# NCKempke/PIPS-IPMpp

Measured on AMD Instinct MI355X. Metric: KKT factor+solve per IPM iter/sec, N-block arrowhead LP, higher is better.
Workload: dtype f64; 1 GPU; 64 blocks x 10000 vars (5000 eq rows, rho=0.001), Schur dim 2000, 64 blocks/GPU [BASELINE configs[1]]; deterministic=False, family=random, root=dense LDL^T, sparse_head=multifrontal (k_front), solves_per_unit=4, collective=none, nnzL_per_gpu=649118456

## Files before the change

include/pips_hip.h:

```cpp
#ifndef PIPS_HIP_H
#define PIPS_HIP_H
#include <stddef.h>
#include <stdint.h>

#ifdef __cplusplus
extern "C" {
#endif

const char* pips_hip_last_error(void);
long long pips_hip_host_wait_count(void);
int pips_hip_host_wait_sites(char* buf, int cap);
long long pips_hip_device_allocs_live(void);
long long pips_hip_device_bytes_live(void);
int pips_hip_device_count(void);

int pips_hip_ldl_create(void** handle, int n, const int* krow, const int* jcol, int device, int flags);
int pips_hip_ldl_set_inertia_hint(void* handle, int n_primal);
int pips_hip_ldl_set_pivot_rule(void* handle, double thr_rel, double repl_rel);
int pips_hip_ldl_set_refinement(void* handle, int max_steps, double tol);
int pips_hip_ldl_set_refinement_backward_error(void* handle, int max_steps, double tol);
int pips_hip_ldl_set_deterministic(void* handle, int on);
int pips_hip_ldl_analyze(void* handle);
int pips_hip_ldl_factor(void* handle, const double* vals_host);
int pips_hip_ldl_solve(void* handle, int nrhs, double* rhs_inout_host, int ld);
// ... 197 lines not shown
int pips_gen_root(uint64_t seed, int n0, int myl, int* F0_rowptr, int* F0_colidx, double* F0_val, double* c0,
                  double* xstar0);
int pips_gen_diagonal(uint64_t seed, int block, int n, double lo, double hi, double* d);
int pips_kkt_leaf_assemble(int nx, int my, int mz, const int* Q_rowptr, const int* Q_colidx, const double* Q_val,
                           const int* B_rowptr, const int* B_colidx, const double* B_val, const int* D_rowptr,
                           const int* D_colidx, const double* D_val, int* K_rowptr, int* K_colidx, double* K_val,
                           int* diag_pos);
int pips_border_assemble(int nx, int my, int mz, int n0, int n_empty, int myl, int mzl, const int* R_rowptr,
                         const int* R_colidx, const double* R_val, const int* A_rowptr, const int* A_colidx,
                         const double* A_val, const int* C_rowptr, const int* C_colidx, const double* C_val,
                         const int* F_rowptr, const int* F_colidx, const double* F_val, const int* G_rowptr,
                         const int* G_colidx, const double* G_val, int* Bt_rowptr, int* Bt_colidx, double* Bt_val);
int pips_map_children_to_ranks(int n_children, int n_ranks, int* map);
int pips_symbolic_probe(int n, int n_primal, const int* krow, const int* jcol, int S, const int* Bt_rowptr,
                        const int* Bt_colidx, int force_n_head, int64_t* what, int n_what, int* perm, int* colcount);

int pips_symbolic_probe_hubs(int n, int n_primal, const int* krow, const int* jcol, int n_hubs, const int* hubs, int min_size,
                             int64_t* what, int n_what, int* perm, int* colcount);

int pips_layout_probe(int nblk, const int* n, const int* n_primal, const int* const* krow, const int* const* kcol,
                      int S, const int* const* bt_rowptr, const int* const* bt_colidx,
                      int deterministic, long long free_device_bytes, int64_t* what, int n_what);

int pips_schur_pack_probe(int nblk, int S, const int* const* bt_rowptr, int* nb, int* nb_max, int* const* local_of_row);

int pips_gdx_read_block(void** block, const char* path, int num_blocks, int act_block, int offset);
int pips_gdx_block_counts(void* block, long long* counts14);
int pips_gdx_block_vector(void* block, int which, double* out, int capacity, int* length);
int pips_gdx_block_matrix(void* block, int which, int* present, int* rows, int* cols, int* rowptr, int* colidx, double* val);
void pips_gdx_block_destroy(void* block);

#ifdef __cplusplus
}
#endif
#endif
```

pips-ipmpp_amd/csrc/engine.hip:

```cpp
#include <hip/hip_runtime.h>

#include <algorithm>
#include <cstdlib>
#include <cstring>
#include <map>
#include <memory>
#include <mutex>
#include <thread>
#include <vector>

#include "common.h"
#include "devmem.h"
#include "layout.h"
#include "kernels.hip.h"
#include "rootkernel.hip.h"
#include "tailkernel.hip.h"
#include "pips_hip.h"

namespace pips {

static thread_local std::string g_last_error;
void set_last_error(const std::string& msg) { g_last_error = msg; }
std::atomic<long long> g_host_waits{0};
struct WaitSite { std::atomic<const char*> file{nullptr}; std::atomic<int> line{0}; std::atomic<long long> n{0}; };
// ... 35 lines not shown
static int env_flag(const char* name) {
   const char* v = getenv(name);
   return v ? (atoi(v) != 0 ? 1 : 0) : -1;
}

static inline int grid_for(long long n, int block, int cap = 4096) {
   long long g = (n + block - 1) / block;
   if (g < 1) g = 1;
   if (g > cap) g = cap;
   return (int)g;
}

struct TaskList { long long off = 0; int cnt = 0; };

struct TailPlan {
   int ntc_max = 0;
   std::vector<TaskList> upd, upd_diag, diag, trsm, fwd, bwd, trail, trail_next;
   TaskList schur;
   DevBuf<TileTask> d_tasks;
   std::vector<TileTask> h_tasks;

   int build(const std::vector<BlkDesc>& blks, int panel = 0, bool lookahead = false, bool split_diag = false,
             const std::vector<const std::vector<int>*>* first = nullptr, bool diag_ahead = false, int pair2 = 1) {
      std::vector<TileTask> all;
      ntc_max = 0;
      for (auto& b : blks) ntc_max = std::max(ntc_max, b.ntc);
      upd.assign(ntc_max, {});
      upd_diag.assign(ntc_max, {});
      diag.assign(ntc_max, {});
      trsm.assign(ntc_max, {});
      fwd.assign(ntc_max, {});
      bwd.assign(ntc_max, {});
      trail.assign(ntc_max, {});
      trail_next.assign(ntc_max, {});
      const int nblk = (int)blks.size();
      auto begin = [&](TaskList& l) { l.off = (long long)all.size(); };
      auto end = [&](TaskList& l) { l.cnt = (int)((long long)all.size() - l.off); };
      for (int j = 0; j < ntc_max; ++j) {
         const int p0 = panel > 0 ? j / panel * panel : 0;
         auto fst = [&](int b, int t) { return first ? (*(*first)[b])[t] : 0; };
         begin(upd_diag[j]);
         if (j > p0 && split_diag)
            for (int b = 0; b < nblk; ++b)
               if (blks[b].ntc > j) {
                  const int k0 = std::max(p0, fst(b, j));
                  if (k0 < j) all.push_back({b, j, j, (diag_ahead ? std::max(k0, j - 1) : k0) | (j << 16)});
// ... 54 lines not shown
         end(bwd[j]);
         if (panel > 0 && (j + 1) % panel == 0) {
            begin(trail_next[j]);
            if (lookahead)
               for (int b = 0; b < nblk; ++b)
                  if (j + 1 < blks[b].ntc)
                     for (int ti = j + 1; ti < blks[b].ntr; ++ti) all.push_back({b, ti, j + 1, p0 | ((j + 1) << 16)});
            end(trail_next[j]);
            begin(trail[j]);
            for (int b = 0; b < nblk; ++b)
               for (int tj = j + (lookahead ? 2 : 1); tj < blks[b].ntc; ++tj)
                  for (int ti = tj; ti < blks[b].ntr; ++ti) all.push_back({b, ti, tj, p0 | ((j + 1) << 16)});
            end(trail[j]);
         }
      }
      begin(schur);
      for (int b = 0; b < nblk; ++b)
         if (blks[b].ntc > 0 && blks[b].nb > 0) {
            const int nt = blks[b].nb_pad / TILE;
            for (int ti = 0; ti < nt; ++ti)
               for (int tj = 0; tj <= ti; ++tj) all.push_back({b, ti, tj, 0});
         }
      end(schur);
      h_tasks = all;
      return d_tasks.upload(all);
   }
};

struct SweepRt {
   DevBuf<TileTask> d_tasks;
   int n_tasks = 0;
   DevBuf<int> d_ints;
   long long n_flags = 0;
   DevBuf<long long> d_flag_off, d_tfirst_off;
   DevBuf<int> d_tfirst;
   int epoch = 0;
   bool enabled = false;
   long long poll_limit = SWEEP_POLL_LIMIT;
   int take_error(const char* who) {
      if (!d_ints) return PIPS_OK;
      int w = 0;
      HIP_TRY(hipMemcpy(&w, d_ints + 2 * SWEEP_NRHS_MAX, sizeof(int), hipMemcpyDeviceToHost));
      if (!w) return PIPS_OK;
      HIP_TRY(hipMemset(d_ints + 2 * SWEEP_NRHS_MAX, 0, sizeof(int)));
      PIPS_FAIL(PIPS_ERR_HIP, "%s: a single-launch solve sweep gave up waiting for a piece of the solution after %lld polls (its output is NaN); "
                              "another process holding the device for seconds can cause that - PIPS_HIP_SWEEP_LAUNCHES=1 selects the launch-per-column sweeps",
                who, poll_limit);
   }
// ... 185 lines not shown
   bool is_root = false;
   const int* d_sctab = nullptr;
   const std::vector<TaskList>* sc_groups = nullptr;
   const TileTask* d_sc_tasks = nullptr;
   const std::vector<hipEvent_t>* ev_sc = nullptr;
   int* d_ctr_pool = nullptr;
   int* ctr_cursor = nullptr;
   const std::vector<TaskList>* det_rounds = nullptr;
   const TileTask* d_det_tasks = nullptr;
   double* d_gbuf = nullptr;
   long long gstride = 0;
   const int* d_blk_group = nullptr;
   int n_groups = 0, first_slot = 0;
   long long sc_len = 0;
   bool det_defer_reduce = false;
   bool det_reduce_later = false;
   bool bunch_kaufman = false;
   int *d_pert_cnt = nullptr, *d_pert_list = nullptr;
   const double* bk_orig = nullptr;
   int bk_orig_ld = 0, bk_orig_rowmajor = 0;
   const int* d_bk_perm = nullptr;
   int bk_isolate = 0;
   const TailSingle* single = nullptr;
};
constexpr int GEMM_CTR_SLOTS = 4096;
constexpr int GEMM_BAL_MIN_TASKS = 1024;

static void reduce_det_groups(const TailCtx& c, double* SC, int ldSC) {
   const int S_ = ldSC;
   if (c.det_defer_reduce) {
   } else if (c.d_sctab)
      hipLaunchKernelGGL(k_reduce_groups, dim3((unsigned)std::max(1LL, std::min(1024LL, (c.sc_len + 255) / 256)), 1), dim3(256), 0, c.stream, SC, 0, (int)c.sc_len,
                         c.d_gbuf, c.gstride, c.n_groups, c.first_slot);
   else
      hipLaunchKernelGGL(k_reduce_groups, dim3(std::max(1, std::min(64, (S_ + 255) / 256)), S_), dim3(256), 0, c.stream, SC, ldSC, S_, c.d_gbuf,
                         c.gstride, c.n_groups, c.first_slot);
}

static inline int tile_grid(int n) { return (n + 7) / 8 * 8; }
template <int MODE>
static void launch_tile_gemm(const TailCtx& c, const TileTask* tasks, const TaskList& l, hipStream_t st, double* SC = nullptr, int ldSC = 0) {
   const bool rounds = MODE == 2 && c.det_rounds;
   hipLaunchKernelGGL(k_tile_gemm<MODE>, dim3(tile_grid(l.cnt)), dim3(512), 0, st, tasks + l.off, l.cnt, c.d_blks, c.d_arena, c.d_dtail, c.d_winv, c.d_bmap, SC, ldSC,
                      MODE == 2 ? c.d_sctab : nullptr, c.d_uarena, rounds ? c.d_gbuf : nullptr, rounds ? c.gstride : 0, rounds ? c.d_blk_group : nullptr);
}
static bool tile_gemm_bal_ready(const TailCtx& c) { return c.d_ctr_pool && *c.ctr_cursor < GEMM_CTR_SLOTS; }
template <int MODE>
static void launch_tile_gemm_bal(const TailCtx& c, const TileTask* tasks, const TaskList& l, hipStream_t st, double* SC = nullptr, int ldSC = 0) {
   const int wgs = tile_grid(l.cnt) / 8 * 9;
   hipLaunchKernelGGL(k_tile_gemm_bal<MODE>, dim3(tile_grid(wgs)), dim3(512), 0, st, tasks + l.off, l.cnt, c.d_blks, c.d_arena, c.d_dtail, c.d_winv, c.d_bmap, SC, ldSC,
                      MODE == 2 ? c.d_sctab : nullptr, c.d_uarena, c.d_ctr_pool + 8 * (*c.ctr_cursor)++);
}
static void launch_tile_diag(const TailCtx& c, const TileTask* tasks, const TaskList& l, hipStream_t st) {
   if (c.bunch_kaufman)
      hipLaunchKernelGGL(k_tile_diag_bk, dim3(l.cnt), dim3(256), 0, st, tasks + l.off, c.d_blks, c.d_arena, c.d_dtail, c.d_winv, c.d_inertia, c.d_pert_cnt, c.d_pert_list,
                         c.bk_orig, c.bk_orig_ld, c.bk_orig_rowmajor, c.d_bk_perm, c.bk_isolate);
   else
      hipLaunchKernelGGL(k_tile_diag, dim3(l.cnt), dim3(256), 0, st, tasks + l.off, c.d_blks, c.d_arena, c.d_dtail, c.d_winv, c.d_psign, c.d_psign_off, c.d_inertia, c.d_pref);
}
static void launch_tile_update(const TailCtx& c, const TaskList& l, hipStream_t st) {
   if (!c.is_root && l.cnt >= GEMM_BAL_MIN_TASKS && tile_gemm_bal_ready(c))
      launch_tile_gemm_bal<0>(c, c.plan->d_tasks, l, st);
   else if (c.is_root)
      launch_tile_gemm<3>(c, c.plan->d_tasks, l, st);
   else
      launch_tile_gemm<0>(c, c.plan->d_tasks, l, st);
}

static int dump_tail_trace(const TailCtx& c, DevBuf<long long>& d_trace, size_t n_trace, const char* trace_file) {
   const TailSingle& ts = *c.single;
   std::vector<long long> h(n_trace);
   std::vector<TileTask> ht((size_t)ts.n_tasks);
   HIP_TRY(hipStreamSynchronize(c.stream));
   HIP_TRY(hipMemcpy(h.data(), d_trace, h.size() * sizeof(long long), hipMemcpyDeviceToHost));
   HIP_TRY(hipMemcpy(ht.data(), ts.d_tasks, ht.size() * sizeof(TileTask), hipMemcpyDeviceToHost));
   d_trace.reset();
   if (FILE* f = fopen(trace_file, "w")) {
      for (int t = 0; t < ts.n_tasks; ++t) {
         int x = 0;
         while (x < 7 && t >= ts.args.xoff[x + 1]) ++x;
         fprintf(f, "%d %d %d %d %d %d %d %lld %lld %lld\n", t, x, ht[t].blk >> 24, ht[t].blk & 0xffffff, ht[t].ti, ht[t].tj, ht[t].pad, h[3 * (size_t)t], h[3 * (size_t)t + 1],
                 h[3 * (size_t)t + 2]);
      }
      fclose(f);
   }
   return PIPS_OK;
}

static int tail_single_launch(const TailCtx& c) {
// ... 51 lines not shown
         else launch_tile_gemm<1>(c, p.d_tasks, p.trsm[j], c.stream);
      }
      if (p.trsm[j].cnt > 0 && c.bunch_kaufman && c.is_root && c.d_pert_cnt)
         hipLaunchKernelGGL(k_bk_growth, dim3(TILE), dim3(256), 0, c.stream, c.d_blks, c.d_arena, j, 1e8, c.d_pert_cnt, c.d_pert_list);
      if (p.trail_next[j].cnt > 0 || p.trail[j].cnt > 0) {
         PIPS_TRY(main_writes(j + 1));
         const bool split = c.side && p.trail[j].cnt > 0;
         if (split) {
            HIP_TRY(hipEventRecord(c.ev_panel, c.stream));
            HIP_TRY(hipStreamWaitEvent(c.side, c.ev_panel, 0));
            launch_tile_update(c, p.trail[j], c.side);
            HIP_TRY(hipEventRecord(c.ev_rest, c.side));
            side_busy = true;
            side_from = j + 2;
         }
         PhaseTimer::Scope phase(c.timer, c.stream, 2);
         if (p.trail_next[j].cnt > 0) launch_tile_update(c, p.trail_next[j], c.stream);
         if (!split && p.trail[j].cnt > 0) launch_tile_update(c, p.trail[j], c.stream);
      }
   }
   return main_writes(1 << 30);
}

static int tail_schur(const TailCtx& c, double* SC, int ldSC) {
   const TailPlan& p = *c.plan;
   const bool rounds = c.det_rounds != nullptr, panels = !rounds && c.sc_groups && !c.d_sctab;
   if (!SC || (!rounds && !panels && p.schur.cnt == 0)) return PIPS_OK;
   PhaseTimer::Scope phase(c.timer, c.stream, 5);
   if (rounds) {
      for (const TaskList& l : *c.det_rounds)
         if (l.cnt > 0) launch_tile_gemm<2>(c, c.d_det_tasks, l, c.stream, SC, ldSC);
      if (!c.det_reduce_later) reduce_det_groups(c, SC, ldSC);
   } else if (panels) {
      for (size_t g = 0; g < c.sc_groups->size(); ++g) {
         const TaskList& l = (*c.sc_groups)[g];
         if (l.cnt > 0) launch_tile_gemm<2>(c, c.d_sc_tasks, l, c.stream, SC, ldSC);
         HIP_TRY(hipEventRecord((*c.ev_sc)[g], c.stream));
      }
   } else if (tile_gemm_bal_ready(c) && !c.d_sctab)
      launch_tile_gemm_bal<2>(c, p.d_tasks, p.schur, c.stream, SC, ldSC);
   else
      launch_tile_gemm<2>(c, p.d_tasks, p.schur, c.stream, SC, ldSC);
   return PIPS_OK;
}

static int tail_factor(const TailCtx& c, double* SC, int ldSC) {
   const bool trsm_tri = !c.bunch_kaufman && !c.is_root && env_int("PIPS_HIP_TRSM_DENSE", 0) == 0;
   if (!c.single) PIPS_TRY(tail_columns(c, trsm_tri));
   else if (c.single->n_tasks > 0) PIPS_TRY(tail_single_launch(c));
   PIPS_TRY(tail_schur(c, SC, ldSC));
   HIP_TRY(hipGetLastError());
   return PIPS_OK;
}

static int tail_fwd(const TailCtx& c, double* xw, int nrhs = 1, long long xw_stride = 0) {
   const TailPlan& p = *c.plan;
   if (c.sweep && c.sweep->enabled && nrhs <= SWEEP_NRHS_MAX) {
      hipLaunchKernelGGL(k_tail_rows_fwd, dim3(c.sweep->n_tasks, nrhs), dim3(256), 0, c.stream, c.sweep->args(xw_stride, c.stream), c.d_blks, c.d_arena, c.d_dtail,
                         c.d_winv, xw);
      HIP_TRY(hipGetLastError());
      return PIPS_OK;
   }
   for (int j = 0; j < p.ntc_max; ++j)
      if (p.fwd[j].cnt > 0)
         hipLaunchKernelGGL(k_tail_fwd, dim3(p.fwd[j].cnt, nrhs), dim3(256), 0, c.stream, p.d_tasks + p.fwd[j].off, c.d_blks,
                            c.d_arena, c.d_dtail, c.d_winv, xw, j, xw_stride);
   HIP_TRY(hipGetLastError());
   return PIPS_OK;
}

static int tail_bwd(const TailCtx& c, double* xw, int nrhs = 1, long long xw_stride = 0, int border = 0) {
// ... 32 lines not shown
   SchurPack pack;
   int packed_rhs = 0;
   DevBuf<int> d_pk_la;
   DevBuf<long long> d_pk_tabrow;
   std::vector<int> h_pk_la, h_pk_tab;
   std::vector<long long> h_pk_tabrow;
   DevBuf<int> d_kb_rec;
   DevBuf<long long> d_kb_off;
   DevBuf<int> d_kb_list;
   DevBuf<int> d_kb_tail;
   DevBuf<double> d_mfU;
   DevBuf<double> d_mfLV;
   DevBuf<int> d_roots, d_root_off;
   DevBuf<BbBatch> d_bb_batches;
   DevBuf<BbMeta> d_bb_meta;
   DevBuf<int> d_bb_off, d_bb_pos;
   DevBuf<double> d_bb_out;
   DevBuf<int> d_bb_round_blk;
   DevBuf<int> d_round_blk;
   DevBuf<int> d_mfint;
   DevBuf<long long> d_mfdbg;
   DevBuf<int> d_spine, d_spine_off;
   TailPlan plan;
   SweepRt sweep;
   TailSingle tsingle;
   DevBuf<double> d_uarena;
   DevBuf<double> d_arena, d_kval, d_bval, d_winv, d_dtail, d_xw, d_rhs, d_res, d_stage, d_pref;
   DevBuf<long long> d_kdst, d_bdst, d_kdiag, d_kptr, d_psign_off, d_perm_off, d_rowbase, d_bt_xoff;
   DevBuf<SnDesc> d_sns;
   DevBuf<BlkDesc> d_blks;
   DevBuf<int> d_lf_rows, d_lf_ptr, d_lf_src, d_lf_pos;
   DevBuf<double> d_lf_val;
   DevBuf<LeafDesc> d_leafdesc;
   DevBuf<int> d_lb_list;
   DevBuf<int> d_rowidx, d_upd, d_sncol, d_bmap, d_perm, d_inertia, d_nprimal;
   DevBuf<int> d_br_rowptr, d_br_sc, d_br_src;
   DevBuf<int> d_krowptr, d_kcolidx, d_bt_rowptr, d_bt_colidx, d_bt_rowsc;
   DevBuf<signed char> d_psign;
   struct GatherList {
      long long n_targets = 0, n_slots = 0;
      DevBuf<long long> d_tgt, d_off, d_slots;
   };
   struct SlotEntry { long long target, slot; };
   DevBuf<double> d_slot_val, d_vslot_val;
   DevBuf<double> d_mvslot;
   std::vector<GatherList> g_levels, gv_levels;
// ... 250 lines not shown
         HIP_TRY(hipEventCreateWithFlags(&ev, hipEventDisableTiming));
         ev_sc.push_back(ev);
      }
      if (all.empty()) all.push_back({-1, 0, 0, 0});
      return d_sc_tasks.upload(all);
   }
   TailCtx ctx() {
      TailCtx c;
      c.d_blks = d_blks; c.plan = &plan; c.d_arena = d_arena; c.d_uarena = d_uarena; c.d_dtail = d_dtail; c.d_winv = d_winv;
      c.d_psign = d_psign; c.d_psign_off = d_psign_off; c.d_inertia = d_inertia; c.d_pref = d_pref;
      c.stream = stream; c.side = side; c.ev_panel = ev_diag_in; c.ev_rest = ev_diag_out; c.d_bmap = d_bmap; c.d_sctab = d_sctab;
      if (!sc_groups.empty()) { c.sc_groups = &sc_groups; c.d_sc_tasks = d_sc_tasks; c.ev_sc = &ev_sc; }
      c.d_ctr_pool = d_gemm_ctr; c.ctr_cursor = &gemm_ctr_cursor;
      if (deterministic && d_gbuf) {
         c.det_rounds = &det_rounds; c.d_det_tasks = d_det_tasks; c.d_gbuf = d_gbuf; c.gstride = det_gstride(); c.sc_len = sc_len; c.d_blk_group = d_blk_group;
         c.n_groups = det_n_groups; c.first_slot = det_first_slot;
         c.det_defer_reduce = det_global && defer_group_reduce;
      }
      c.sweep = &sweep;
      if (tail_single) {
         tsingle.args.blks = d_blks; tsingle.args.arena = d_arena; tsingle.args.uarena = d_uarena; tsingle.args.winv = d_winv; tsingle.args.dtail = d_dtail;
         tsingle.args.pref = d_pref; tsingle.args.psign = d_psign; tsingle.args.psign_off = d_psign_off; tsingle.args.inertia = d_inertia;
         c.single = &tsingle;
      }
      return c;
   }

   int analyze(int n_threads) {
      for (int b = 0; b < nblk; ++b)
         if (in[b].n <= 0) PIPS_FAIL(PIPS_ERR_STATE, "pips_hip_batch_analyze: block %d was never set", b);
      AnalyzeKnobs knobs;
      read_layout_knobs(this, opt, knobs);
      HIP_TRY(hipSetDevice(device));
      release();
      {
         size_t free_b = 0, total_b = 0;
         (void)hipMemGetInfo(&free_b, &total_b);
         knobs.free_device_bytes = (long long)free_b;
      }
      int rc = analyze_symbolic(in, S, n_threads, opt, knobs, sym);
      if (rc) return rc;
      {
         BatchLayout lay;
         if ((rc = build_batch_layout(in, sym, S, knobs, lay))) return rc;
         static_cast<BatchLayout&>(*this) = std::move(lay);
      }
      if ((rc = upload_layout())) return rc;
      const int pair2 = 4;
      if ((rc = plan.build(h_blks, 0, false, true, &tile_first, true, pair2))) return rc;
      if ((rc = sweep.build(h_blks, &tile_first))) return rc;
      if (tail_single) {
         if ((rc = tsingle.build(plan, h_blks, stream))) return rc;
         tsingle.args.poll_limit = knobs.tail_poll_limit;
         tsingle.args.diag_blocked = knobs.tail_diag_blocked;
      }
      drop_uploaded();
      if (!side) {
         int prio_lo = 0, prio_hi = 0;
         HIP_TRY(hipDeviceGetStreamPriorityRange(&prio_lo, &prio_hi));
         HIP_TRY(hipStreamCreateWithPriority(&side, hipStreamNonBlocking, prio_hi));
         HIP_TRY(hipEventCreateWithFlags(&ev_diag_in, hipEventDisableTiming));
         HIP_TRY(hipEventCreateWithFlags(&ev_diag_out, hipEventDisableTiming));
      }
      h_inertia.assign(3 * nblk, 0);
      analyzed = true;
      ++analysis_gen;
      if (deterministic) {
         if (slots_total + vslots_total > HEAD_SLOTS_MAX)
            PIPS_FAIL(PIPS_ERR_STATE, "deterministic mode: %lld head contributions exceed the slot budget of %lld", slots_total + vslots_total, HEAD_SLOTS_MAX);
         if ((rc = build_deterministic(n_threads))) return rc;
         head_slots = true;
         if ((rc = set_det_groups(0, 1))) return rc;
      }
      return PIPS_OK;
   }

   int upload_layout() {
      if (mf) {
// ... 2647 lines not shown
   if (!hub_dissected_order(n, ap, ai, hv, min_size, pv, cc)) PIPS_FAIL(PIPS_ERR_STATE, "pips_symbolic_probe_hubs: no separators");
   AnalyzeOptions opt;
   AnalyzeKnobs knobs;
   read_layout_knobs(nullptr, opt, knobs);
   opt.mf_konly = false;
   opt.user_perm = pv.data();
   opt.user_colcount = cc.data();
   {
      int cut = 0;
      while (cut < n - n_hubs && cc[cut] <= ROOT_ND_MAX_COLCOUNT) ++cut;
      opt.force_n_head = cut;
   }
   CsrPattern K{n, n, krow, jcol};
   CsrPattern B{0, n, nullptr, nullptr};
   std::vector<BlockSym> sym(1);
   int rc = analyze_block(K, B, n_primal, opt, sym[0]);
   if (rc) return rc;
   if (what) sym_info(sym, what, n_what);
   if (perm) std::copy(sym[0].perm.begin(), sym[0].perm.end(), perm);
   if (colcount) std::copy(sym[0].colcount.begin(), sym[0].colcount.end(), colcount);
   return PIPS_OK;
}

int pips_layout_probe(int nblk, const int* n, const int* n_primal, const int* const* krow, const int* const* kcol, int S,
                      const int* const* bt_rowptr, const int* const* bt_colidx, int deterministic, long long free_device_bytes,
                      int64_t* what, int n_what) {
   if (nblk <= 0 || !n || !krow || !kcol || S < 0) PIPS_FAIL(PIPS_ERR_ARG, "pips_layout_probe: bad arguments");
   std::vector<BlockInput> in(nblk);
   for (int b = 0; b < nblk; ++b) {
      if (n[b] <= 0 || !krow[b] || !kcol[b]) PIPS_FAIL(PIPS_ERR_ARG, "pips_layout_probe: block %d is empty", b);
      in[b].n = n[b];
      in[b].n_primal = n_primal ? n_primal[b] : -1;
      in[b].krow.assign(krow[b], krow[b] + n[b] + 1);
      in[b].kcol.assign(kcol[b], kcol[b] + krow[b][n[b]]);
      if (S > 0 && bt_rowptr && bt_colidx && bt_rowptr[b] && bt_colidx[b]) {
         in[b].btrow.assign(bt_rowptr[b], bt_rowptr[b] + S + 1);
         in[b].btcol.assign(bt_colidx[b], bt_colidx[b] + bt_rowptr[b][S]);
         in[b].btval.assign(in[b].btcol.size(), 0.0);
      }
   }
   AnalyzeOptions opt;
   AnalyzeKnobs knobs;
   read_layout_knobs(nullptr, opt, knobs);
   if (deterministic) { knobs.deterministic = true; opt.mf_konly = false; }
   knobs.free_device_bytes = free_device_bytes;
   std::vector<BlockSym> sym;
   BatchLayout lay;
   const int n_threads = (int)std::max(1u, std::min(16u, std::thread::hardware_concurrency()));
   int rc = analyze_symbolic(in, S, n_threads, opt, knobs, sym);
   if (!rc) rc = build_batch_layout(in, sym, S, knobs, lay);
   if (!rc) rc = check_batch_layout(in, sym, S, knobs, lay);
   if (rc) return rc;
   int64_t v[21] = {lay.arena_total, lay.xw_total, lay.uarena_total, lay.nsn_total, (int64_t)lay.levels.size(), (int64_t)lay.levels_top.size(),
                    (int64_t)lay.mf_launches.size(), 0, lay.n_bb, lay.bb_stage, lay.tail_single, lay.border_backward_ok, lay.aug_sweeps_ok,
                    lay.slots_total, lay.vslots_total, lay.n_total, lay.mf, lay.schur_mode_eff, lay.bb_doubles, lay.mfU_total, lay.spine_total};
   for (const MfLaunch& m : lay.mf_launches) if (m.cls >= 6) v[7] += m.cnt;
   for (int i = 0; what && i < n_what && i < 21; ++i) what[i] = v[i];
   return PIPS_OK;
}

}
```

pips-ipmpp_amd/csrc/kernels.hip.h:

```cpp
#pragma once
#include <hip/hip_runtime.h>
#include <stdint.h>

#include "records.h"

namespace pips {

constexpr int KB = 16;
constexpr int LDS_PAD = 16;
constexpr int LDSW = TILE + LDS_PAD;

typedef double double4_t __attribute__((ext_vector_type(4)));

struct BelowRow { const double* p; long long stride; };
__device__ __forceinline__ BelowRow below_row(const double* __restrict__ arena, const SnDesc& sn, int a) {
   if (a < sn.ld - sn.w) return BelowRow{arena + sn.panel + sn.w + a, (long long)sn.ld};
   return BelowRow{arena + sn.bb + (a - sn.rb), (long long)((sn.r - sn.rb + 3) & ~3)};
}

__device__ __forceinline__ void atomic_add_f64(double* p, double v) {
   __hip_atomic_fetch_add(p, v, __ATOMIC_RELAXED, __HIP_MEMORY_SCOPE_AGENT);
}

struct ScatterCtx {
// ... 1421 lines not shown
                                                         const int* __restrict__ sctab, double* __restrict__ uarena,
                                                         int* __restrict__ ctr) {
   __shared__ GemmShared sh;
   __shared__ int s_tix;
   if (threadIdx.x == 0) {
      const int per = (n_tasks + 7) >> 3;
      const int xcc = (int)(__builtin_amdgcn_s_getreg((3 << 11) | 20 ) & 7);
      int got = -1;
      for (int d = 0; d < 8 && got < 0; ++d) {
         const int x = (xcc + d) & 7;
         if (__hip_atomic_load(ctr + x, __ATOMIC_RELAXED, __HIP_MEMORY_SCOPE_AGENT) >= per) continue;
         const int t = __hip_atomic_fetch_add(ctr + x, 1, __ATOMIC_RELAXED, __HIP_MEMORY_SCOPE_AGENT);
         const int tix = x * per + t;
         if (t < per && tix < n_tasks) got = tix;
      }
      s_tix = got;
   }
   __syncthreads();
   const int tix = s_tix;
   if (tix < 0) return;
   tile_gemm_body<MODE>(tix, sh, tasks, n_tasks, blks, arena, dtail, winv, bmap, SC, ldSC, sctab, uarena);
}

__global__ void k_reduce_groups(double* __restrict__ SC, int ld, int S, const double* __restrict__ gbuf, long long gstride, int n_groups,
                                int first_slot) {
   const int c = blockIdx.y;
   for (int r = c + blockIdx.x * blockDim.x + threadIdx.x; r < S; r += gridDim.x * blockDim.x) {
      const long long off = r + (long long)c * ld;
      double p[8];
#pragma unroll
      for (int g = 0; g < 8; ++g) {
         const int lg = g - first_slot;
         p[g] = (lg >= 0 && lg < n_groups) ? gbuf[lg * gstride + off] : 0.0;
      }
      SC[off] += ((p[0] + p[1]) + (p[2] + p[3])) + ((p[4] + p[5]) + (p[6] + p[7]));
   }
}



struct DiagShared {
   double colk[2][TILE];
   double xrow[2][TILE];
   double dk[TILE];
   double prs[TILE];
   int sgn[TILE];
// ... 1772 lines not shown
```

pips-ipmpp_amd/csrc/records.h:

```cpp
#pragma once
#include <stdint.h>

#ifdef __HIPCC__
#define PIPS_HD __host__ __device__
#else
#define PIPS_HD
#endif

namespace pips {

constexpr int TILE = 128;

struct SnDesc {
   long long panel;
   long long rows;
   long long upd;
   int w, r, c0, blk;
   int n_useg, rb;
   int ld, pad_;
   long long slot;
   long long vslot;
   long long U;
   long long mf;
   long long bb;
};

struct BlkDesc {
   long long arena_off;
   long long T;
   long long sncol_off;
   long long xw_off;
   long long x_off;
   long long bmap_off;
   long long winv_off;
   long long dt_off;
   long long sctab_off;
   int n, n_head, m, m_pad, nb, nb_pad, ldT, ntc, ntr;
   int mf_split;
   long long U;
   double thr_rel, repl_rel;
   double repl_abs;
   long long lv_off;
   long long k_off, b_off;
   long long T_in;
};

struct TileTask { int blk, ti, tj, pad; };

constexpr int HEAD_WMAX = 32;
constexpr int SIMPLE_RMAX = 16;

constexpr int BB_GMAX = 8;
constexpr int BB_TR = 4;
PIPS_HD inline int bb_tile_count(int rp) {
   const int nt4 = rp >> 2;
   if (BB_TR == 4) return nt4 * (nt4 + 1) / 2;
   const int nt8 = (rp + 7) >> 3;
   int cnt = 0;
   for (int tb = 0; tb < nt4; ++tb) cnt += nt8 - (tb >> 1);
   return cnt;
}
struct BbMeta { int lt_off, pos_off, w, nbj, tile0, pad0, pad1, pad2; };
struct BbBatch {
   long long src;
   long long pos;
   int first, cnt;
   int ndoubles, ntiles, npos, pad;
};

struct LeafDesc {
// ... 16 lines not shown
```

pips-ipmpp_amd/python/capi.py:

```python
import ctypes as C
import sys
import os

import numpy as np

try:
    import torch
except Exception:
    torch = None

_HERE = os.path.dirname(os.path.abspath(__file__))
LIB_PATH = os.environ.get("PIPS_HIP_LIBRARY") or os.path.join(os.path.dirname(_HERE), "libpipship.so")


class PipsHipError(RuntimeError):
    pass


def _load():
    if not os.path.exists(LIB_PATH):
        raise PipsHipError(
            f"{LIB_PATH} is missing: build it with `python -c 'import __graft_entry__ as g; g.build()'` "
            "(hipcc --offload-arch=gfx950). The MI355X backend has no CPU fallback.")
    return C.CDLL(LIB_PATH, mode=C.RTLD_GLOBAL)


lib = _load()

_i32p = np.ctypeslib.ndpointer(dtype=np.int32, flags="C_CONTIGUOUS")
_f64p = np.ctypeslib.ndpointer(dtype=np.float64, flags="C_CONTIGUOUS")
_i64p = np.ctypeslib.ndpointer(dtype=np.int64, flags="C_CONTIGUOUS")
_vp = C.c_void_p

lib.pips_hip_last_error.restype = C.c_char_p
lib.pips_hip_device_count.restype = C.c_int
lib.pips_hip_host_wait_count.restype = C.c_longlong
lib.pips_hip_device_allocs_live.restype = C.c_longlong
lib.pips_hip_device_bytes_live.restype = C.c_longlong

SYMBOLS = [
    "pips_hip_last_error", "pips_hip_device_count",
    "pips_hip_ldl_create", "pips_hip_ldl_set_inertia_hint", "pips_hip_ldl_set_pivot_rule", "pips_hip_ldl_set_refinement", "pips_hip_ldl_set_refinement_backward_error", "pips_hip_ldl_set_deterministic",
    "pips_hip_ldl_analyze", "pips_hip_ldl_factor", "pips_hip_ldl_solve", "pips_hip_ldl_inertia", "pips_hip_ldl_info",
    "pips_hip_ldl_get_perm", "pips_hip_ldl_set_border", "pips_hip_ldl_factor_schur", "pips_hip_ldl_destroy",
    "pips_hip_ldl_solve_dev", "pips_hip_ldl_solve_sparse", "pips_hip_ldl_factor_schur_batch", "pips_hip_ldl_solve_batch", "pips_hip_ldl_solve_batch_dev",
    "pips_hip_ldl_inertia_batch",
    "pips_hip_dense_ldl_create", "pips_hip_dense_ldl_factor", "pips_hip_dense_ldl_factor_dev", "pips_hip_dense_ldl_solve",
    "pips_hip_dense_ldl_solve_dev", "pips_hip_dense_ldl_inertia", "pips_hip_dense_ldl_set_pivoting", "pips_hip_dense_ldl_set_distributed", "pips_hip_dense_ldl_destroy", "pips_root_plan_build", "pips_layout_probe", "pips_hip_host_wait_count", "pips_hip_host_wait_sites", "pips_hip_device_allocs_live", "pips_hip_device_bytes_live",
    "pips_hip_batch_create", "pips_hip_batch_set_block", "pips_hip_batch_set_options", "pips_hip_batch_set_schur_mode", "pips_hip_batch_set_deterministic", "pips_hip_batch_get_schur_mode", "pips_hip_batch_add_regularization", "pips_hip_batch_set_refinement",
    "pips_hip_batch_last_refinement_steps", "pips_hip_batch_set_refinement_backward_error",
    "pips_hip_batch_last_refinement_measure", "pips_hip_batch_analyze",
    "pips_hip_batch_set_values", "pips_hip_batch_set_diagonals_dev", "pips_hip_batch_set_diagonals", "pips_hip_batch_factor",
    "pips_hip_batch_solve_dev", "pips_hip_batch_solve", "pips_hip_batch_border_tmult_dev", "pips_hip_batch_border_mult_dev",
    "pips_hip_batch_inertia", "pips_hip_batch_tail_to_host", "pips_hip_batch_info", "pips_hip_batch_sync", "pips_hip_batch_set_timing",
    "pips_hip_batch_get_timing", "pips_hip_batch_destroy",
    "pips_hip_kkt_create", "pips_hip_kkt_create_sparse", "pips_hip_kkt_get_schur_sparse", "pips_hip_kkt_sparse_root_info", "pips_hip_kkt_factorize", "pips_hip_kkt_set_root_regularization", "pips_hip_kkt_solve_compressed", "pips_hip_kkt_get_schur",
    "pips_hip_kkt_set_root_inequalities", "pips_hip_kkt_set_zdiag0_dev", "pips_hip_kkt_set_root_hessian",
    "pips_hip_kkt_root_inertia", "pips_hip_kkt_get_timing", "pips_hip_kkt_last_ltsolve_from_factor", "pips_hip_kkt_last_solve_path", "pips_hip_kkt_set_solve_check", "pips_hip_kkt_solve_check_counts", "pips_hip_kkt_set_solve_graph", "pips_hip_kkt_set_root_stream", "pips_hip_kkt_solve_graph_stats", "pips_hip_kkt_set_root_pivoting", "pips_hip_kkt_destroy",
    "pips_hip_malloc", "pips_hip_free", "pips_hip_memcpy_h2d", "pips_hip_memcpy_d2h", "pips_hip_memset",
    "pips_hip_comm_unique_id", "pips_hip_comm_create", "pips_hip_comm_create_external", "pips_hip_comm_set_external_rsag", "pips_hip_comm_set_external_broadcast", "pips_hip_broadcast", "pips_hip_comm_has_broadcast", "pips_hip_allreduce_sum_rsag", "pips_hip_all_gather", "pips_hip_comm_size", "pips_hip_allreduce_sum", "pips_hip_comm_destroy",
    "pips_hip_vec_axpy", "pips_hip_vec_axpby", "pips_hip_vec_scale", "pips_hip_vec_copy", "pips_hip_vec_set",
    "pips_hip_vec_add_const", "pips_hip_vec_mul", "pips_hip_vec_div", "pips_hip_vec_add_product", "pips_hip_vec_add_quotient",
    "pips_hip_vec_divide_some", "pips_hip_vec_select_nonzeros", "pips_hip_vec_safe_invert", "pips_hip_vec_gondzio_projection", "pips_hip_vec_dot",
    "pips_hip_vec_one_norm", "pips_hip_vec_inf_norm", "pips_hip_vec_min", "pips_hip_vec_sumsq_scaled", "pips_hip_vec_stepbound",
    "pips_hip_vec_find_blocking", "pips_hip_vec_weighted_stepbounds", "pips_hip_vec_dot_shifted", "pips_ipm_create", "pips_ipm_create_rank", "pips_ipm_create_general", "pips_ipm_create_general_scaled", "pips_ipm_create_qp", "pips_ipm_hessian_mult", "pips_ipm_get_scaling", "pips_ipm_get_dims", "pips_ipm_get_iterate", "pips_ipm_get_stats2", "pips_ipm_get_schur_mode", "pips_ipm_mult", "pips_ipm_outer_solve", "pips_ipm_solve", "pips_ipm_set_gondzio", "pips_ipm_set_option", "pips_ipm_set_free_variables", "pips_ipm_get_solution", "pips_ipm_get_trace", "pips_ipm_get_stats", "pips_ipm_destroy",
    "pips_gdx_read_block", "pips_gdx_block_counts", "pips_gdx_block_vector", "pips_gdx_block_matrix", "pips_gdx_block_destroy",
    "pips_gen_row_nnz", "pips_gen_block", "pips_gen_root", "pips_gen_diagonal", "pips_kkt_leaf_assemble",
    "pips_border_assemble", "pips_symbolic_probe", "pips_symbolic_probe_hubs", "pips_map_children_to_ranks", "pips_schur_pack_probe",
]

PIPS_SCALER_NONE = 0
# ... 1040 lines not shown
```

Measured before the change: 8.425 64-block work units/s (1 factorize + 4 solveCompressed).

## Group tail factor columns into panels with side-stream overlap and strip kernels

Adds a PanelPlan that regroups the per-column tile update and TRSM tasks into panels of P columns. Within a panel, updates are applied column by column on the side stream. Trailing updates further down are either launched as one deep GEMM concurrently on the main stream or merged into per-row strips, which a new k_tile_panel kernel runs sequentially inside one workgroup. This targets the many small per-column launches and the serialization of the tail factorization. In exchange it adds a more complex task ordering, cross-stream event dependencies, and strips that run serially in one workgroup, which can leave the GPU under-occupied. It also adds a probe API that exports both task orderings.

After: 8.536 64-block work units/s (1 factorize + 4 solveCompressed), median of 6. 1.3% higher.

```diff
diff --git a/include/pips_hip.h b/include/pips_hip.h
--- a/include/pips_hip.h
+++ b/include/pips_hip.h
@@ -243,6 +243,10 @@
                       int S, const int* const* bt_rowptr, const int* const* bt_colidx,
                       int deterministic, long long free_device_bytes, int64_t* what, int n_what);
 
+int pips_tail_plan_probe(int nblk, const int* n, const int* n_primal, const int* const* krow, const int* const* kcol,
+                         int S, const int* const* bt_rowptr, const int* const* bt_colidx, int force_n_head,
+                         int* col_tasks, long long col_cap, int* grp_tasks, long long grp_cap, int64_t* counts);
+
 int pips_schur_pack_probe(int nblk, int S, const int* const* bt_rowptr, int* nb, int* nb_max, int* const* local_of_row);
 
 int pips_gdx_read_block(void** block, const char* path, int num_blocks, int act_block, int offset);
diff --git a/pips-ipmpp_amd/csrc/engine.hip b/pips-ipmpp_amd/csrc/engine.hip
--- a/pips-ipmpp_amd/csrc/engine.hip
+++ b/pips-ipmpp_amd/csrc/engine.hip
@@ -81,6 +81,11 @@
 
    int build(const std::vector<BlkDesc>& blks, int panel = 0, bool lookahead = false, bool split_diag = false,
              const std::vector<const std::vector<int>*>* first = nullptr, bool diag_ahead = false, int pair2 = 1) {
+      lists(blks, panel, lookahead, split_diag, first, diag_ahead, pair2);
+      return d_tasks.upload(h_tasks);
+   }
+   void lists(const std::vector<BlkDesc>& blks, int panel, bool lookahead, bool split_diag, const std::vector<const std::vector<int>*>* first,
+              bool diag_ahead, int pair2) {
       std::vector<TileTask> all;
       ntc_max = 0;
       for (auto& b : blks) ntc_max = std::max(ntc_max, b.ntc);
@@ -181,8 +186,80 @@
                for (int tj = 0; tj <= ti; ++tj) all.push_back({b, ti, tj, 0});
          }
       end(schur);
-      h_tasks = all;
-      return d_tasks.upload(all);
+      h_tasks = std::move(all);
+   }
+};
+
+struct PanelPlan {
+   int P = 0, n_groups = 0;
+   std::vector<TaskList> deep, pre, block_deep, strips;
+   std::vector<TaskList> upd_in, trsm_in;
+   std::vector<TileTask> h_tasks;
+   std::vector<TileStrip> h_strips;
+   DevBuf<TileTask> d_tasks;
+   DevBuf<TileStrip> d_strips;
+   void lists(const TailPlan& p, int P_) {
+      *this = PanelPlan();
+      P = P_;
+      n_groups = (p.ntc_max + P - 1) / P;
+      struct Group { std::vector<TileTask> deep, pre, block_deep; std::map<std::pair<int, int>, std::vector<TileTask>> strips; };
+      std::vector<Group> gs(n_groups);
+      std::vector<std::vector<TileTask>> ui(p.ntc_max), ti(p.ntc_max);
+      auto each = [&](const TaskList& l, auto&& f) {
+         for (long long q = l.off; q < l.off + l.cnt; ++q)
+            if (p.h_tasks[q].blk >= 0) f(p.h_tasks[q]);
+      };
+      auto update = [&](const TileTask& t) {
+         const int k1 = t.pad >> 16, g = k1 / P * P;
+         if (t.ti >= g + P) {
+            if (k1 == g) gs[g / P].deep.push_back(t);
+            else if (t.ti == t.tj) gs[t.tj / P].pre.push_back(t);
+            else gs[g / P].strips[{t.blk, t.ti}].push_back(t);
+         } else if (k1 == g)
+            gs[g / P].block_deep.push_back(t);
+         else
+            ui[k1].push_back(t);
+      };
+      for (int j = 0; j < p.ntc_max; ++j) {
+         each(p.upd_diag[j], update);
+         each(p.upd[j], update);
+         each(p.trsm[j], [&](const TileTask& t) {
+            const int g = j / P * P;
+            if (t.ti >= g + P) gs[g / P].strips[{t.blk, t.ti}].push_back(t);
+            else ti[j].push_back(t);
+         });
+      }
+      auto put = [&](TaskList& l, const std::vector<TileTask>& v) {
+         l.off = (long long)h_tasks.size(); l.cnt = (int)v.size();
+         h_tasks.insert(h_tasks.end(), v.begin(), v.end());
+      };
+      deep.assign(n_groups, {}); pre.assign(n_groups, {}); block_deep.assign(n_groups, {}); strips.assign(n_groups, {});
+      upd_in.assign(p.ntc_max, {}); trsm_in.assign(p.ntc_max, {});
+      auto step = [](const TileTask& t) { return t.pad ? 2 * (t.pad >> 16) : 2 * t.tj + 1; };
+      for (int i = 0; i < n_groups; ++i) {
+         put(deep[i], gs[i].deep);
+         put(pre[i], gs[i].pre);
+         put(block_deep[i], gs[i].block_deep);
+         strips[i].off = (long long)h_strips.size();
+         for (auto& kv : gs[i].strips) {
+            std::vector<TileTask>& v = kv.second;
+            std::stable_sort(v.begin(), v.end(), [&](const TileTask& a, const TileTask& b) { return step(a) != step(b) ? step(a) < step(b) : a.tj < b.tj; });
+            h_strips.push_back({(int)h_tasks.size(), (int)v.size()});
+            h_tasks.insert(h_tasks.end(), v.begin(), v.end());
+         }
+         strips[i].cnt = (int)((long long)h_strips.size() - strips[i].off);
+         for (int j = i * P; j < std::min((i + 1) * P, p.ntc_max); ++j) {
+            put(upd_in[j], ui[j]);
+            put(trsm_in[j], ti[j]);
+         }
+      }
+   }
+   int build(const TailPlan& p, int P_) {
+      lists(p, P_);
+      if (h_tasks.empty()) h_tasks.push_back({-1, 0, 0, 0});
+      if (h_strips.empty()) h_strips.push_back({0, 0});
+      PIPS_TRY(d_tasks.upload(h_tasks));
+      return d_strips.upload(h_strips);
    }
 };
 
@@ -414,6 +491,7 @@
    const int* d_bk_perm = nullptr;
    int bk_isolate = 0;
    const TailSingle* single = nullptr;
+   const PanelPlan* panels = nullptr;
 };
 constexpr int GEMM_CTR_SLOTS = 4096;
 constexpr int GEMM_BAL_MIN_TASKS = 1024;
@@ -450,13 +528,14 @@
    else
       hipLaunchKernelGGL(k_tile_diag, dim3(l.cnt), dim3(256), 0, st, tasks + l.off, c.d_blks, c.d_arena, c.d_dtail, c.d_winv, c.d_psign, c.d_psign_off, c.d_inertia, c.d_pref);
 }
-static void launch_tile_update(const TailCtx& c, const TaskList& l, hipStream_t st) {
+static void launch_tile_update(const TailCtx& c, const TaskList& l, hipStream_t st, const TileTask* tasks = nullptr) {
+   if (!tasks) tasks = c.plan->d_tasks;
    if (!c.is_root && l.cnt >= GEMM_BAL_MIN_TASKS && tile_gemm_bal_ready(c))
-      launch_tile_gemm_bal<0>(c, c.plan->d_tasks, l, st);
+      launch_tile_gemm_bal<0>(c, tasks, l, st);
    else if (c.is_root)
-      launch_tile_gemm<3>(c, c.plan->d_tasks, l, st);
+      launch_tile_gemm<3>(c, tasks, l, st);
    else
-      launch_tile_gemm<0>(c, c.plan->d_tasks, l, st);
+      launch_tile_gemm<0>(c, tasks, l, st);
 }
 
 static int dump_tail_trace(const TailCtx& c, DevBuf<long long>& d_trace, size_t n_trace, const char* trace_file) {
@@ -554,6 +633,39 @@
    return main_writes(1 << 30);
 }
 
+static int tail_panels(const TailCtx& c) {
+   const TailPlan& p = *c.plan;
+   const PanelPlan& g = *c.panels;
+   const int n_tasks = (int)g.h_tasks.size();
+   for (int i = 0; i < g.n_groups; ++i) {
+      const bool beside = g.deep[i].cnt > 0;
+      const hipStream_t st = beside ? c.side : c.stream;
+      PhaseTimer* const tm = beside ? nullptr : c.timer;
+      if (beside) {
+         HIP_TRY(hipEventRecord(c.ev_panel, c.stream));
+         HIP_TRY(hipStreamWaitEvent(c.side, c.ev_panel, 0));
+      }
+      if (g.pre[i].cnt > 0) { PhaseTimer::Scope phase(tm, st, 2); launch_tile_gemm<4>(c, g.d_tasks, g.pre[i], st); }
+      if (g.block_deep[i].cnt > 0) { PhaseTimer::Scope phase(tm, st, 2); launch_tile_gemm<4>(c, g.d_tasks, g.block_deep[i], st); }
+      for (int j = i * g.P; j < std::min((i + 1) * g.P, p.ntc_max); ++j) {
+         if (g.upd_in[j].cnt > 0) { PhaseTimer::Scope phase(tm, st, 2); launch_tile_gemm<4>(c, g.d_tasks, g.upd_in[j], st); }
+         { PhaseTimer::Scope phase(tm, st, 3); launch_tile_diag(c, p.d_tasks, p.diag[j], st); }
+         if (g.trsm_in[j].cnt > 0) { PhaseTimer::Scope phase(tm, st, 4); launch_tile_gemm<5>(c, g.d_tasks, g.trsm_in[j], st); }
+      }
+      if (beside) {
+         HIP_TRY(hipEventRecord(c.ev_rest, c.side));
+         { PhaseTimer::Scope phase(c.timer, c.stream, 2); launch_tile_update(c, g.deep[i], c.stream, g.d_tasks); }
+         HIP_TRY(hipStreamWaitEvent(c.stream, c.ev_rest, 0));
+      }
+      if (g.strips[i].cnt > 0) {
+         PhaseTimer::Scope phase(c.timer, c.stream, 2);
+         hipLaunchKernelGGL(k_tile_panel, dim3(tile_grid(g.strips[i].cnt)), dim3(512), 0, c.stream, g.d_strips + g.strips[i].off, g.strips[i].cnt, g.d_tasks, n_tasks,
+                            c.d_blks, c.d_arena, c.d_dtail, c.d_winv, c.d_uarena);
+      }
+   }
+   return PIPS_OK;
+}
+
 static int tail_schur(const TailCtx& c, double* SC, int ldSC) {
    const TailPlan& p = *c.plan;
    const bool rounds = c.det_rounds != nullptr, panels = !rounds && c.sc_groups && !c.d_sctab;
@@ -578,7 +690,8 @@
 
 static int tail_factor(const TailCtx& c, double* SC, int ldSC) {
    const bool trsm_tri = !c.bunch_kaufman && !c.is_root && env_int("PIPS_HIP_TRSM_DENSE", 0) == 0;
-   if (!c.single) PIPS_TRY(tail_columns(c, trsm_tri));
+   if (!c.single && c.panels && c.side && trsm_tri && env_int("PIPS_HIP_TAIL_PANEL", 1) != 0) PIPS_TRY(tail_panels(c));
+   else if (!c.single) PIPS_TRY(tail_columns(c, trsm_tri));
    else if (c.single->n_tasks > 0) PIPS_TRY(tail_single_launch(c));
    PIPS_TRY(tail_schur(c, SC, ldSC));
    HIP_TRY(hipGetLastError());
@@ -657,6 +770,7 @@
    DevBuf<long long> d_mfdbg;
    DevBuf<int> d_spine, d_spine_off;
    TailPlan plan;
+   PanelPlan panels;
    SweepRt sweep;
    TailSingle tsingle;
    DevBuf<double> d_uarena;
@@ -953,7 +1067,8 @@
          tsingle.args.blks = d_blks; tsingle.args.arena = d_arena; tsingle.args.uarena = d_uarena; tsingle.args.winv = d_winv; tsingle.args.dtail = d_dtail;
          tsingle.args.pref = d_pref; tsingle.args.psign = d_psign; tsingle.args.psign_off = d_psign_off; tsingle.args.inertia = d_inertia;
          c.single = &tsingle;
-      }
+      } else if (panels.n_groups > 0)
+         c.panels = &panels;
       return c;
    }
 
@@ -984,7 +1099,8 @@
          if ((rc = tsingle.build(plan, h_blks, stream))) return rc;
          tsingle.args.poll_limit = knobs.tail_poll_limit;
          tsingle.args.diag_blocked = knobs.tail_diag_blocked;
-      }
+      } else if ((rc = panels.build(plan, pair2)))
+         return rc;
       drop_uploaded();
       if (!side) {
          int prio_lo = 0, prio_hi = 0;
@@ -3678,13 +3794,12 @@
    return PIPS_OK;
 }
 
-int pips_layout_probe(int nblk, const int* n, const int* n_primal, const int* const* krow, const int* const* kcol, int S,
-                      const int* const* bt_rowptr, const int* const* bt_colidx, int deterministic, long long free_device_bytes,
-                      int64_t* what, int n_what) {
-   if (nblk <= 0 || !n || !krow || !kcol || S < 0) PIPS_FAIL(PIPS_ERR_ARG, "pips_layout_probe: bad arguments");
-   std::vector<BlockInput> in(nblk);
+static int probe_inputs(const char* who, int nblk, const int* n, const int* n_primal, const int* const* krow, const int* const* kcol, int S,
+                        const int* const* bt_rowptr, const int* const* bt_colidx, std::vector<BlockInput>& in) {
+   if (nblk <= 0 || !n || !krow || !kcol || S < 0) PIPS_FAIL(PIPS_ERR_ARG, "%s: bad arguments", who);
+   in.assign(nblk, BlockInput());
    for (int b = 0; b < nblk; ++b) {
-      if (n[b] <= 0 || !krow[b] || !kcol[b]) PIPS_FAIL(PIPS_ERR_ARG, "pips_layout_probe: block %d is empty", b);
+      if (n[b] <= 0 || !krow[b] || !kcol[b]) PIPS_FAIL(PIPS_ERR_ARG, "%s: block %d is empty", who, b);
       in[b].n = n[b];
       in[b].n_primal = n_primal ? n_primal[b] : -1;
       in[b].krow.assign(krow[b], krow[b] + n[b] + 1);
@@ -3695,6 +3810,14 @@
          in[b].btval.assign(in[b].btcol.size(), 0.0);
       }
    }
+   return PIPS_OK;
+}
+
+int pips_layout_probe(int nblk, const int* n, const int* n_primal, const int* const* krow, const int* const* kcol, int S,
+                      const int* const* bt_rowptr, const int* const* bt_colidx, int deterministic, long long free_device_bytes,
+                      int64_t* what, int n_what) {
+   std::vector<BlockInput> in;
+   PIPS_TRY(probe_inputs("pips_layout_probe", nblk, n, n_primal, krow, kcol, S, bt_rowptr, bt_colidx, in));
    AnalyzeOptions opt;
    AnalyzeKnobs knobs;
    read_layout_knobs(nullptr, opt, knobs);
@@ -3715,4 +3838,68 @@
    return PIPS_OK;
 }
 
-}
+int pips_tail_plan_probe(int nblk, const int* n, const int* n_primal, const int* const* krow, const int* const* kcol, int S,
+                         const int* const* bt_rowptr, const int* const* bt_colidx, int force_n_head, int* col_tasks, long long col_cap,
+                         int* grp_tasks, long long grp_cap, int64_t* counts) {
+   std::vector<BlockInput> in;
+   PIPS_TRY(probe_inputs("pips_tail_plan_probe", nblk, n, n_primal, krow, kcol, S, bt_rowptr, bt_colidx, in));
+   if (!counts || col_cap < 0 || grp_cap < 0 || (col_cap > 0 && !col_tasks) || (grp_cap > 0 && !grp_tasks))
+      PIPS_FAIL(PIPS_ERR_ARG, "pips_tail_plan_probe: bad arguments");
+   AnalyzeOptions opt;
+   AnalyzeKnobs knobs;
+   read_layout_knobs(nullptr, opt, knobs);
+   opt.force_n_head = force_n_head;
+   knobs.free_device_bytes = 0;
+   std::vector<BlockSym> sym;
+   BatchLayout lay;
+   const int n_threads = (int)std::max(1u, std::min(16u, std::thread::hardware_concurrency()));
+   PIPS_TRY(analyze_symbolic(in, S, n_threads, opt, knobs, sym));
+   PIPS_TRY(build_batch_layout(in, sym, S, knobs, lay));
+   TailPlan plan;
+   plan.lists(lay.h_blks, 0, false, true, &lay.tile_first, true, 4);
+   PanelPlan pp;
+   pp.lists(plan, 4);
+   long long nc = 0, ng = 0, launches_col = 0, launches_grp = 0;
+   auto col = [&](const TaskList& l, int kind) {
+      launches_col += l.cnt > 0;
+      for (long long q = l.off; q < l.off + l.cnt; ++q, ++nc) {
+         const TileTask& t = plan.h_tasks[q];
+         if (nc < col_cap) { int* r = col_tasks + 6 * nc; r[0] = kind; r[1] = t.blk; r[2] = t.ti; r[3] = t.tj; r[4] = t.pad & 0xffff; r[5] = t.pad >> 16; }
+      }
+   };
+   auto grp = [&](long long off, int cnt, int list, int group, int index) {
+      for (int q = 0; q < cnt; ++q, ++ng) {
+         const TileTask& t = pp.h_tasks[off + q];
+         if (ng < grp_cap) {
+            int* r = grp_tasks + 9 * ng;
+            r[0] = list; r[1] = group; r[2] = index; r[3] = q; r[4] = t.blk; r[5] = t.ti; r[6] = t.tj; r[7] = t.pad & 0xffff; r[8] = t.pad >> 16;
+         }
+      }
+   };
+   auto grp_list = [&](const TaskList& l, int list, int group, int index) { launches_grp += l.cnt > 0; grp(l.off, l.cnt, list, group, index); };
+   for (int j = 0; j < plan.ntc_max; ++j) {
+      col(plan.upd_diag[j], 0);
+      col(plan.upd[j], 0);
+      launches_col += plan.diag[j].cnt > 0;
+      col(plan.trsm[j], 1);
+   }
+   for (int i = 0; i < pp.n_groups; ++i) {
+      grp_list(pp.deep[i], 0, i, 0);
+      grp_list(pp.pre[i], 1, i, 0);
+      grp_list(pp.block_deep[i], 2, i, 0);
+      for (int j = i * pp.P; j < std::min((i + 1) * pp.P, plan.ntc_max); ++j) {
+         grp_list(pp.upd_in[j], 3, i, j);
+         launches_grp += plan.diag[j].cnt > 0;
+         grp_list(pp.trsm_in[j], 4, i, j);
+      }
+      launches_grp += pp.strips[i].cnt > 0;
+      for (int q = 0; q < pp.strips[i].cnt; ++q) {
+         const TileStrip& st = pp.h_strips[pp.strips[i].off + q];
+         grp(st.off, st.cnt, 5, i, q);
+      }
+   }
+   counts[0] = nc; counts[1] = ng; counts[2] = plan.ntc_max; counts[3] = pp.n_groups; counts[4] = launches_col; counts[5] = launches_grp;
+   return PIPS_OK;
+}
+
+}
diff --git a/pips-ipmpp_amd/csrc/kernels.hip.h b/pips-ipmpp_amd/csrc/kernels.hip.h
--- a/pips-ipmpp_amd/csrc/kernels.hip.h
+++ b/pips-ipmpp_amd/csrc/kernels.hip.h
@@ -1467,6 +1467,29 @@
    tile_gemm_body<MODE>(tix, sh, tasks, n_tasks, blks, arena, dtail, winv, bmap, SC, ldSC, sctab, uarena);
 }
 
+__global__ __launch_bounds__(512, 4) void k_tile_panel(const TileStrip* __restrict__ strips, int n_strips, const TileTask* __restrict__ tasks,
+                                                      int n_tasks, const BlkDesc* __restrict__ blks, double* __restrict__ arena,
+                                                      const double* __restrict__ dtail, const double* __restrict__ winv,
+                                                      double* __restrict__ uarena) {
+   __shared__ GemmShared sh;
+   const int per = (n_strips + 7) >> 3;
+   const int six = (int)(blockIdx.x & 7) * per + (int)(blockIdx.x >> 3);
+   if (six >= n_strips) return;
+   const TileStrip s = strips[six];
+   for (int t = s.off; t < s.off + s.cnt; ++t) {
+      if (t > s.off) {
+         dma_wait();
+         __builtin_amdgcn_fence(__ATOMIC_RELEASE, "workgroup");
+         __syncthreads();
+         __builtin_amdgcn_fence(__ATOMIC_ACQUIRE, "workgroup");
+      }
+      if (__builtin_amdgcn_readfirstlane(tasks[t].pad) == 0)
+         tile_gemm_body<5>(t, sh, tasks, n_tasks, blks, arena, dtail, winv, nullptr, nullptr, 0, nullptr, uarena);
+      else
+         tile_gemm_body<0>(t, sh, tasks, n_tasks, blks, arena, dtail, winv, nullptr, nullptr, 0, nullptr, uarena);
+   }
+}
+
 __global__ void k_reduce_groups(double* __restrict__ SC, int ld, int S, const double* __restrict__ gbuf, long long gstride, int n_groups,
                                 int first_slot) {
    const int c = blockIdx.y;
diff --git a/pips-ipmpp_amd/csrc/records.h b/pips-ipmpp_amd/csrc/records.h
--- a/pips-ipmpp_amd/csrc/records.h
+++ b/pips-ipmpp_amd/csrc/records.h
@@ -46,6 +46,7 @@
 };
 
 struct TileTask { int blk, ti, tj, pad; };
+struct TileStrip { int off, cnt; };
 
 constexpr int HEAD_WMAX = 32;
 constexpr int SIMPLE_RMAX = 16;
diff --git a/pips-ipmpp_amd/python/capi.py b/pips-ipmpp_amd/python/capi.py
--- a/pips-ipmpp_amd/python/capi.py
+++ b/pips-ipmpp_amd/python/capi.py
@@ -46,7 +46,7 @@
     "pips_hip_ldl_solve_dev", "pips_hip_ldl_solve_sparse", "pips_hip_ldl_factor_schur_batch", "pips_hip_ldl_solve_batch", "pips_hip_ldl_solve_batch_dev",
     "pips_hip_ldl_inertia_batch",
     "pips_hip_dense_ldl_create", "pips_hip_dense_ldl_factor", "pips_hip_dense_ldl_factor_dev", "pips_hip_dense_ldl_solve",
-    "pips_hip_dense_ldl_solve_dev", "pips_hip_dense_ldl_inertia", "pips_hip_dense_ldl_set_pivoting", "pips_hip_dense_ldl_set_distributed", "pips_hip_dense_ldl_destroy", "pips_root_plan_build", "pips_layout_probe", "pips_hip_host_wait_count", "pips_hip_host_wait_sites", "pips_hip_device_allocs_live", "pips_hip_device_bytes_live",
+    "pips_hip_dense_ldl_solve_dev", "pips_hip_dense_ldl_inertia", "pips_hip_dense_ldl_set_pivoting", "pips_hip_dense_ldl_set_distributed", "pips_hip_dense_ldl_destroy", "pips_root_plan_build", "pips_layout_probe", "pips_tail_plan_probe", "pips_hip_host_wait_count", "pips_hip_host_wait_sites", "pips_hip_device_allocs_live", "pips_hip_device_bytes_live",
     "pips_hip_batch_create", "pips_hip_batch_set_block", "pips_hip_batch_set_options", "pips_hip_batch_set_schur_mode", "pips_hip_batch_set_deterministic", "pips_hip_batch_get_schur_mode", "pips_hip_batch_add_regularization", "pips_hip_batch_set_refinement",
     "pips_hip_batch_last_refinement_steps", "pips_hip_batch_set_refinement_backward_error",
     "pips_hip_batch_last_refinement_measure", "pips_hip_batch_analyze",
```
